# NUSTM/FacialMMT

Hardware: AMD Instinct MI355X
Metric: utterances/sec T+A+V forward+bwd, 160-frame face seq, 1/2/4/8 GPU (higher is better)
Workload: dtype bf16; 1 GPU; configs[1]: T+A+V, RoBERTa-large (random init), 160-frame face seq (uint8 112x112 crops, fused pil-bicubic x2 + normalise), batch 4 utterances/GPU, bf16, fwd+bwd+clip+AdamW every step; global_batch=4, parallelism=dp1, hip_graphs=whole step: 2 graphs (fwd+bwd | clip+optimizer), text_encoder_concurrent_with_swin=True, swin_forward_pipelined_across_steps=False, text_encoder_parameters=bf16 with fp32 master weights in the optimizer

## Files before the change

### facialmmt_amd/_lib.py

```python
from __future__ import annotations

import ctypes as C
import os

_HERE = os.path.dirname(os.path.abspath(__file__))
LIB_PATH = os.path.join(_HERE, "libfmmt_hip.so")

F32, BF16 = 0, 1
GENERIC = 0x100
EPI_NONE, EPI_GELU, EPI_GELU_BWD, EPI_GELU_DG, EPI_MUL_AUX = 0, 1, 2, 3, 4
SAVE_DG = 0x200
BATCH_MAJOR = 0x400
RESIZE_PIL, RESIZE_CV2 = 0, 1

_p, _i, _f, _sz, _u64 = C.c_void_p, C.c_int, C.c_float, C.c_size_t, C.c_uint64

SIGNATURES = {
    "fmmt_version": (_i, []),
    "fmmt_linear_fwd": (_i, [_i, _i, _i, _i, _p, _i, _p, _i, _p, _p, _i, _p, _i, _p, _i, _p, _i, _p, _i, _p]),
    "fmmt_linear_splitk_workspace": (_sz, [_i, _i, _i]),
    "fmmt_linear_fwd_splitk": (_i, [_i, _i, _i, _i, _p, _i, _p, _i, _p, _p, _i, _p, _sz, _p]),
    "fmmt_linear_wgrad_workspace": (_sz, [_i, _i, _i, _i]),
    "fmmt_linear_wgrad": (_i, [_i, _i, _i, _i, _p, _i, _p, _i, _p, _p, _p, _i, _i, _p, _sz, _p]),
    "fmmt_linear_wgrad_partials": (_i, [_i, _i, _i, _i, _p, _i, _p, _i, _i, _p, _i, _i, _p, _sz, _p]),
# ... 108 lines not shown

GROUPS_SIGNATURES = {
    "fmmt_adamw_groups": (_i, [_i, _i, _p, _i, _p, _p, _p, _p, _f, _i, _p]),
    "fmmt_adamw_groups_guarded": (_i, [_i, _i, _p, _i, _p, _p, _p, _p, _f, _i, _p]),
}
ADAMW_GROUP_BYTES = 32
ADAMW_GROUP_FIELDS = [("lr", "<u8"), ("beta1", "<f4"), ("beta2", "<f4"), ("eps", "<f4"), ("weight_decay", "<f4"), ("pad", "<u4", (2,))]

STATS_SIGNATURES = {
    "fmmt_table_stats": (_i, [_i, _i, _i, _p, _p, _p, _p, _p, _p, _p]),
}
STATS_G, STATS_P, STATS_M, STATS_V = 0, 1, 2, 3
STATS_BYTES, STATS_BAD_WORDS = 16, 2
STATS_FIELDS = [("sumsq", "<f4"), ("max_abs", "<f4"), ("nonfinite", "<i4"), ("reserved", "<i4")]

TOKENS_SIGNATURES = {
    "fmmt_token_layout": (_i, [_i, _i, _i, _p, _p, _p, _p, _p, _p, _p]),
    "fmmt_unpack_rows": (_i, [_i, _i, _i, _sz, _p, _p, _p, _p]),
    "fmmt_mha_fwd_ragged": (_i, [_i, _i, _i, _i, _i, _i, _p, _p, _p, _i, _p, _p, _i, _f, _f, _u64, _p, _p, _i, _p, _p]),
    "fmmt_mha_bwd_ragged": (_i, [_i, _i, _i, _i, _i, _i, _p, _p, _p, _i, _p, _p, _i, _f, _f, _u64, _p, _p, _p, _i, _p, _p, _i, _p, _p, _i, _p]),
    "fmmt_dropadd_ln_fwd_map": (_i, [_i, _i, _i, _f, _p, _p, _p, _p, _f, _u64, _p, _u64, _p, _p, _p, _p]),
    "fmmt_dropadd_ln_bwd_map": (_i, [_i, _i, _i, _f, _p, _p, _p, _f, _u64, _p, _u64, _p, _p, _p, _p, _p, _p, _sz, _p, _p]),
}
LOSS_SIGNATURES = {
    "fmmt_ce_fwd": (_i, [_i, _i, _i, _p, _i, _p, _p, _f, _p, _p, _p]),
    "fmmt_ce_bwd": (_i, [_i, _i, _i, _p, _i, _p, _p, _f, _p, _p, _p, _i, _p]),
    "fmmt_pool_head_fwd_crit": (_i, [_i, _i, _i, _i, _i, _p, _p, _p, _p, _p, _p, _p, _p, _p, _f, _u64, _p, _p, _p, _p, _p, _p, _p, _f, _p, _p, _sz, _p]),
    "fmmt_pool_head_bwd_crit": (_i, [_i, _i, _i, _i, _i, _p, _p, _p, _p, _p, _p, _p, _p, _p, _p, _p, _p, _f, _p, _p, _p, _p, _p, _p, _p, _p, _p, _sz, _p]),
}
ROUTE_SIGNATURES = {
    "fmmt_linear_fwd_route": (_i, [_i] * 17),
    "fmmt_linear_wgrad_route": (_i, [_i] * 10),
}
ROUTE_MODE_FWD, ROUTE_MODE_SEG3_N, ROUTE_MODE_SEG3_K, ROUTE_MODE_SPLITK = 0, 1, 2, 3
CE_MAXNL, CE_MAXB = 8, 65536
RAGGED = 0x800

FMMT_EINVAL, FMMT_EALIGN, FMMT_EWORKSPACE = -1, -2, -3
_ERR = {-1: "FMMT_EINVAL (bad shape / unsupported size)", -2: "FMMT_EALIGN (pointer or leading dimension not 16-byte aligned)",
        -3: "FMMT_EWORKSPACE (workspace too small)"}

_lib = None


class FmmtError(RuntimeError):
    pass


def load():
    global _lib
    if _lib is not None:
        return _lib
    if not os.path.exists(LIB_PATH):
        raise FmmtError(f"{LIB_PATH} is missing: build it with `python -m facialmmt_amd.build` "
                        f"(or __graft_entry__.build()); there is no CPU / PyTorch fallback for the hot path")
    lib = C.CDLL(LIB_PATH)
    for name, (res, args) in list(SIGNATURES.items()) + list(POOL_HEAD_SIGNATURES.items()) + list(RAGGED_SIGNATURES.items()) + list(EVAL_COLLECT_SIGNATURES.items()) + list(POOL_HEAD_ROWS_SIGNATURES.items()) + list(GUARD_SIGNATURES.items()) + list(DIGEST_SIGNATURES.items()) + list(EVAL_SHARD_SIGNATURES.items()) + list(JITTER_SIGNATURES.items()) + list(AUG_SIGNATURES.items()) + list(GROUPS_SIGNATURES.items()) + list(STATS_SIGNATURES.items()) + list(TOKENS_SIGNATURES.items()) + list(LOSS_SIGNATURES.items()) + list(ROUTE_SIGNATURES.items()):
        fn = getattr(lib, name)
        fn.restype = res
        fn.argtypes = args
    _lib = lib
    return lib


def check(rc: int, what: str):
    if rc != 0:
        msg = _ERR.get(rc, f"hipError_t {rc}")
        raise FmmtError(f"{what} failed: {msg}")


def dtype_code(t) -> int:
    import torch
    if t == torch.float32:
        return F32
    if t == torch.bfloat16:
        return BF16
    raise FmmtError(f"unsupported activation dtype {t}: the HIP path computes in float32 (parity) or bfloat16 (throughput)")
```

### facialmmt_amd/build.py

```python
from __future__ import annotations

import glob
import os
import subprocess
import sys
from concurrent.futures import ThreadPoolExecutor

HERE = os.path.dirname(os.path.abspath(__file__))
CSRC = os.path.join(HERE, "csrc")
OUT = os.path.join(HERE, "libfmmt_hip.so")
SOURCES = ["gemm.hip", "layernorm.hip", "attn.hip", "wattn_mfma.hip", "wattn_bwd_ref.hip", "wblock.hip", "wblock_ref.hip", "mha_mfma.hip", "misc.hip", "preproc.hip", "mlp_fused.hip", "mlp_ref.hip", "patch_ln.hip", "lin_lnbwd.hip", "plm_fused.hip", "frame_filter.hip", "eval.hip", "pool_head.hip", "ragged.hip", "guard.hip", "digest.hip", "eval_shard.hip", "color_jitter.hip", "aff_augment.hip", "adamw_groups.hip", "table_stats.hip", "ce_loss.hip"]
FLAGS = ["--offload-arch=gfx950", "-O3", "-std=c++17", "-fPIC", "-ffp-contract=fast"]


def _stale(target, deps):
    if not os.path.exists(target):
        return True
    t = os.path.getmtime(target)
    return any(os.path.getmtime(d) > t for d in deps)


def build(force: bool = False, verbose: bool = True, tag: str = "") -> str:
    hipcc = os.environ.get("HIPCC", "/opt/rocm/bin/hipcc")
    tag = tag or os.environ.get("FMMT_BUILD_TAG", "")
    csrc = os.environ.get("FMMT_CSRC_DIR", CSRC) if tag else CSRC
    headers = sorted(glob.glob(os.path.join(csrc, "*.h"))) + [os.path.join(csrc, "..", "..", "include", h) for h in ("fmmt.h", "fmmt_pool_head.h", "fmmt_ragged.h", "fmmt_eval_collect.h", "fmmt_pool_head_rows.h", "fmmt_guard.h", "fmmt_digest.h", "fmmt_eval_shard.h", "fmmt_jitter.h", "fmmt_aug.h", "fmmt_groups.h", "fmmt_stats.h", "fmmt_tokens.h", "fmmt_loss.h", "fmmt_route.h")]
    objdir = os.path.join(HERE, "build_" + tag if tag else "build")
    out = os.path.join(HERE, f"libfmmt_hip_{tag}.so") if tag else OUT
    os.makedirs(objdir, exist_ok=True)
    jobs = []
    for s in SOURCES:
        src = os.path.join(csrc, s)
        obj = os.path.join(objdir, s.replace(".hip", ".o"))
        if force or _stale(obj, [src] + headers):
            jobs.append((src, obj))

    def cc(job):
        src, obj = job
        cmd = [hipcc] + FLAGS + os.environ.get("FMMT_CFLAGS", "").split() + ["-c", src, "-o", obj]
        if verbose:
            print(" ".join(cmd), flush=True)
        subprocess.run(cmd, check=True)

    with ThreadPoolExecutor(max_workers=4) as ex:
        list(ex.map(cc, jobs))
    objs = [os.path.join(objdir, s.replace(".hip", ".o")) for s in SOURCES]
    if force or jobs or _stale(out, objs):
        cmd = [hipcc, "--offload-arch=gfx950", "-shared", "-fPIC", "-o", out] + objs
        if verbose:
            print(" ".join(cmd), flush=True)
        subprocess.run(cmd, check=True)
    return out


if __name__ == "__main__":
    print(build(force="--force" in sys.argv))
```

### facialmmt_amd/csrc/misc.hip

```cpp
#include "fmmt_common.h"
#include "bn1d_core.h"
#include "adamw_core.h"
#include "../../include/fmmt.h"

namespace {

constexpr int IMG = 224, PS = 4, GRID = 56, KPATCH = 48;

template <typename T, bool TO_COLS>
__global__ void patch_cols_kernel(const T* __restrict__ src, T* __restrict__ dst, size_t total) {
    const size_t t = (size_t)blockIdx.x * blockDim.x + threadIdx.x;
    if (t >= total) return;
    const int px = (int)(t % GRID);
    size_t r = t / GRID;
    const int y = (int)(r % IMG);
    r /= IMG;
    const int c = (int)(r % 3);
    const size_t n = r / 3;
    const size_t img_off = ((n * 3 + c) * IMG + y) * IMG + (size_t)px * PS;
    const size_t col_off = ((n * GRID + (y >> 2)) * GRID + px) * KPATCH + c * 16 + (y & 3) * PS;
    const T* s = TO_COLS ? src + img_off : src + col_off;
    T* d = TO_COLS ? dst + col_off : dst + img_off;
    if constexpr (sizeof(T) == 2) *reinterpret_cast<uint2*>(d) = *reinterpret_cast<const uint2*>(s);
    else *reinterpret_cast<uint4*>(d) = *reinterpret_cast<const uint4*>(s);
// ... 147 lines not shown
    }
#pragma unroll
    for (int i = 0; i < 4; ++i) {
        const int r = tr * 64 + ty + 16 * i;
#pragma unroll
        for (int j = 0; j < 4; ++j) {
            const int c = tc * 64 + tx + 16 * j;
            if (r < d.rows && c < d.cols) {
                const size_t o = (size_t)r * d.src_ld + c;
                const bf16 v = f32 ? (bf16)sf[o] : sb[o];
                if (tp) tile[ty + 16 * i][tx + 16 * j] = v;
                else dst[(size_t)r * d.cols + c] = v;
            }
        }
    }
    if (!tp) return;
    __syncthreads();
#pragma unroll
    for (int i = 0; i < 4; ++i) {
        const int c = tc * 64 + ty + 16 * i;
#pragma unroll
        for (int j = 0; j < 4; ++j) {
            const int r = tr * 64 + tx + 16 * j;
            if (r < d.rows && c < d.cols) dst[(size_t)c * d.rows + r] = tile[tx + 16 * j][ty + 16 * i];
        }
    }
}

struct HoDesc {
    const void* src; float* dst;
    long long n;
    int blk_begin, flags;
};
__global__ __launch_bounds__(256) void grad_handover_kernel(const HoDesc* __restrict__ desc, int n_desc, float* __restrict__ partial) {
    __shared__ float red[4];
    int lo = 0, hi = n_desc - 1;
    while (lo < hi) {
        const int mid = (lo + hi + 1) >> 1;
        if (desc[mid].blk_begin <= (int)blockIdx.x) lo = mid;
        else hi = mid - 1;
    }
    const HoDesc d = desc[lo];
    const long long base = (long long)((int)blockIdx.x - d.blk_begin) * 4096;
    const bool bf = d.flags & 1, acc = d.flags & 2;
    const float* sf = reinterpret_cast<const float*>(d.src);
    const bf16* sb = reinterpret_cast<const bf16*>(d.src);
    float ss = 0.f;
    const bool vec = base + 4096 <= d.n && ((reinterpret_cast<uintptr_t>(d.src) | reinterpret_cast<uintptr_t>(d.dst)) & 15) == 0;
    if (vec) {
#pragma unroll
        for (int i = 0; i < 4; ++i) {
            const long long o = base + (long long)(i * 256 + threadIdx.x) * 4;
            f32x4 v;
            if (bf) {
                const bf16x4 t = *reinterpret_cast<const bf16x4*>(sb + o);
#pragma unroll
                for (int e = 0; e < 4; ++e) v[e] = (float)t[e];
            } else {
                v = *reinterpret_cast<const f32x4*>(sf + o);
            }
            if (acc) v += *reinterpret_cast<const f32x4*>(d.dst + o);
            *reinterpret_cast<f32x4*>(d.dst + o) = v;
#pragma unroll
            for (int e = 0; e < 4; ++e) ss += v[e] * v[e];
        }
    } else {
        for (long long o = base + threadIdx.x; o < base + 4096 && o < d.n; o += 256) {
            float v = bf ? (float)sb[o] : sf[o];
            if (acc) v += d.dst[o];
            d.dst[o] = v;
            ss += v * v;
        }
    }
    ss = wave_sum(ss);
    if ((threadIdx.x & 63) == 0) red[threadIdx.x >> 6] = ss;
    __syncthreads();
    if (threadIdx.x == 0) partial[blockIdx.x] = (red[0] + red[1]) + (red[2] + red[3]);
}
__global__ __launch_bounds__(1024) void sumsq_finish_kernel(const float* __restrict__ partial, int n, float* __restrict__ out) {
    __shared__ float red[1024];
    float a = 0.f;
    int i = threadIdx.x;
    for (; i + 7 * 1024 < n; i += 8 * 1024) {
        float v[8];
#pragma unroll
        for (int u = 0; u < 8; ++u) v[u] = partial[i + u * 1024];
#pragma unroll
        for (int u = 0; u < 8; ++u) a += v[u];
    }
    for (; i < n; i += 1024) a += partial[i];
    red[threadIdx.x] = a;
    __syncthreads();
    for (int s = 512; s > 0; s >>= 1) {
        if ((int)threadIdx.x < s) red[threadIdx.x] += red[threadIdx.x + s];
        __syncthreads();
    }
    if (threadIdx.x == 0) out[0] = sqrtf(red[0]);
}

__global__ __launch_bounds__(256) void adamw_batch_kernel(const AdamDesc* __restrict__ desc, int n_desc, const float* __restrict__ lr_p,
                                                          const float* __restrict__ step_p, const float* __restrict__ norm_p,
                                                          float beta1, float beta2, float eps, float wd, float max_norm, int hf) {
    const int r = adamw_find_record(desc, n_desc);
    adamw_batch_body<false>(desc[r], AdamHyper{*lr_p, beta1, beta2, eps, wd}, step_p, norm_p, max_norm, hf);
}

__global__ __launch_bounds__(256) void lnp_bwd_kernel(int M, int C, float eps, const bf16* __restrict__ dy, const bf16* __restrict__ x,
                                                      const bf16* __restrict__ gamma, bf16* __restrict__ dx, float* __restrict__ part) {
    constexpr int MAXV = 4;
    __shared__ float red[4][2][64 * 8];
// ... 188 lines not shown
    const int vec = dtype == FMMT_BF16 ? 8 : 4;
    if (N % vec || ldx % vec) return FMMT_EINVAL;
    if ((reinterpret_cast<uintptr_t>(x) & 15) != 0) return FMMT_EALIGN;
    hipStream_t st = reinterpret_cast<hipStream_t>(stream);
    const dim3 grid((unsigned)((N + 4 * vec - 1) / (4 * vec)));
    if (dtype == FMMT_BF16) {
        if (out_dtype == FMMT_BF16) hipLaunchKernelGGL((colsum_kernel<bf16, bf16>), grid, dim3(256), 0, st, M, N, (const bf16*)x, ldx, (bf16*)out);
        else hipLaunchKernelGGL((colsum_kernel<bf16, float>), grid, dim3(256), 0, st, M, N, (const bf16*)x, ldx, (float*)out);
    } else {
        hipLaunchKernelGGL((colsum_kernel<float, float>), grid, dim3(256), 0, st, M, N, (const float*)x, ldx, (float*)out);
    }
    FMMT_CHECK_LAUNCH();
    return 0;
}

extern "C" int fmmt_cast_batch(int n_desc, int n_tiles, const void* desc, void* stream) {
    if (n_desc <= 0 || n_tiles <= 0 || !desc) return FMMT_EINVAL;
    hipLaunchKernelGGL(cast_batch_kernel, dim3((unsigned)n_tiles), dim3(256), 0, reinterpret_cast<hipStream_t>(stream),
                       reinterpret_cast<const CastDesc*>(desc), n_desc);
    FMMT_CHECK_LAUNCH();
    return 0;
}

extern "C" int fmmt_grad_handover(int n_desc, int n_blocks, const void* desc, float* partial, float* norm_out, void* stream) {
    if (n_desc <= 0 || n_blocks <= 0 || !desc || !partial || !norm_out) return FMMT_EINVAL;
    hipStream_t st = reinterpret_cast<hipStream_t>(stream);
    hipLaunchKernelGGL(grad_handover_kernel, dim3((unsigned)n_blocks), dim3(256), 0, st, reinterpret_cast<const HoDesc*>(desc), n_desc, partial);
    FMMT_CHECK_LAUNCH();
    hipLaunchKernelGGL(sumsq_finish_kernel, dim3(1), dim3(1024), 0, st, (const float*)partial, n_blocks, norm_out);
    FMMT_CHECK_LAUNCH();
    return 0;
}

extern "C" int fmmt_adamw_batch(int n_desc, int n_blocks, const void* desc, const float* lr, const float* step, const float* total_norm,
                                float beta1, float beta2, float eps, float weight_decay, float max_norm, int hf_semantics, void* stream) {
    if (n_desc <= 0 || n_blocks <= 0 || !desc || !lr || !step) return FMMT_EINVAL;
    hipLaunchKernelGGL(adamw_batch_kernel, dim3((unsigned)n_blocks), dim3(256), 0, reinterpret_cast<hipStream_t>(stream),
                       reinterpret_cast<const AdamDesc*>(desc), n_desc, lr, step, total_norm, beta1, beta2, eps, weight_decay, max_norm, hf_semantics);
    FMMT_CHECK_LAUNCH();
    return 0;
}

extern "C" size_t fmmt_layernorm_bwd_bf16_workspace(int M, int C) {
    if (M <= 0 || C <= 0) return 0;
    const int blocks = M / 4 < 1 ? 1 : (M / 4 > 256 ? 256 : M / 4);
    return (size_t)blocks * 2 * (size_t)C * sizeof(float);
}

extern "C" int fmmt_layernorm_bwd_bf16(int M, int C, float eps, const void* dy, const void* x, const void* gamma, void* dx,
                                       void* dgamma, void* dbeta, void* workspace, size_t workspace_bytes, void* stream) {
    if (M <= 0 || C <= 0 || C % 8 || C > 2048) return FMMT_EINVAL;
    if (!dy || !x || !gamma || !dx || !dgamma || !dbeta || !workspace) return FMMT_EINVAL;
    if (workspace_bytes < fmmt_layernorm_bwd_bf16_workspace(M, C)) return FMMT_EWORKSPACE;
    if (((reinterpret_cast<uintptr_t>(dy) | reinterpret_cast<uintptr_t>(x) | reinterpret_cast<uintptr_t>(gamma) | reinterpret_cast<uintptr_t>(dx)) & 15) != 0)
        return FMMT_EALIGN;
    hipStream_t st = reinterpret_cast<hipStream_t>(stream);
    const int blocks = M / 4 < 1 ? 1 : (M / 4 > 256 ? 256 : M / 4);
    hipLaunchKernelGGL(lnp_bwd_kernel, dim3(blocks), dim3(256), 0, st, M, C, eps, (const bf16*)dy, (const bf16*)x, (const bf16*)gamma, (bf16*)dx,
                       reinterpret_cast<float*>(workspace));
    FMMT_CHECK_LAUNCH();
    hipLaunchKernelGGL(lnp_reduce_kernel, dim3((2 * C + 31) / 32), dim3(1024), 0, st, reinterpret_cast<const float*>(workspace), blocks, C,
                       (bf16*)dgamma, (bf16*)dbeta);
    FMMT_CHECK_LAUNCH();
    return 0;
}
```

### facialmmt_amd/ops.py

```python
from __future__ import annotations

import math
import weakref

import torch
from torch.autograd import Function

from . import _lib
from ._lib import EPI_GELU, EPI_GELU_BWD, EPI_GELU_DG, EPI_MUL_AUX, EPI_NONE, SAVE_DG, check, dtype_code


def _st():
    return torch.cuda.current_stream().cuda_stream


def _p(t):
    return None if t is None else t.data_ptr()


def _c16(t: torch.Tensor) -> torch.Tensor:
    t = t.contiguous()
    return t.clone() if t.data_ptr() % 16 else t


# ... 275 lines not shown

def adamw_batch_guarded(n, blocks, desc, lr, step, total_norm, beta1, beta2, eps, weight_decay, max_norm, hf=False):
    if total_norm is None:
        raise ValueError("adamw_batch_guarded: total_norm is what the guard decides on; it cannot be None")
    check(_lib.load().fmmt_adamw_batch_guarded(n, blocks, _p(desc), _p(lr), _p(step), _p(total_norm), float(beta1), float(beta2), float(eps),
                                               float(weight_decay), float(max_norm), 1 if hf else 0, _st()), "fmmt_adamw_batch_guarded")


def _group_tables(n, n_groups, group_of, groups, what):
    if group_of.dtype != torch.int32 or not group_of.is_contiguous() or group_of.numel() != n:
        raise ValueError(f"{what}: group_of is a contiguous int32 tensor with one entry per descriptor record ({n})")
    if groups.dtype != torch.uint8 or not groups.is_contiguous() or groups.numel() != n_groups * _lib.ADAMW_GROUP_BYTES or n_groups < 1:
        raise ValueError(f"{what}: groups is a contiguous uint8 tensor of n_groups >= 1 records of {_lib.ADAMW_GROUP_BYTES} bytes (include/fmmt_groups.h)")
    return _p(group_of), _p(groups)


def adamw_groups(n, blocks, desc, n_groups, group_of, groups, step, total_norm, max_norm, hf=False):
    go, gr = _group_tables(n, n_groups, group_of, groups, "adamw_groups")
    check(_lib.load().fmmt_adamw_groups(n, blocks, _p(desc), n_groups, go, gr, _p(step), _p(total_norm), float(max_norm), 1 if hf else 0, _st()),
          "fmmt_adamw_groups")


def adamw_groups_guarded(n, blocks, desc, n_groups, group_of, groups, step, total_norm, max_norm, hf=False):
    if total_norm is None:
        raise ValueError("adamw_groups_guarded: total_norm is what the guard decides on; it cannot be None")
    go, gr = _group_tables(n, n_groups, group_of, groups, "adamw_groups_guarded")
    check(_lib.load().fmmt_adamw_groups_guarded(n, blocks, _p(desc), n_groups, go, gr, _p(step), _p(total_norm), float(max_norm), 1 if hf else 0,
                                                _st()), "fmmt_adamw_groups_guarded")


def grad_handover_raw(n, blocks, table, partial, norm_out):
    check(_lib.load().fmmt_grad_handover(n, blocks, _p(table), _p(partial), _p(norm_out), torch.cuda.current_stream(table.device).cuda_stream),
          f"fmmt_grad_handover(n={n},blocks={blocks})")


def _guard_words(words):
    if words.dtype != torch.int64 or not words.is_contiguous() or words.numel() != _lib.GUARD_WORDS:
        raise ValueError(f"words: a contiguous int64 tensor of {_lib.GUARD_WORDS} entries (include/fmmt_guard.h)")
    return _p(words)


def guard_commit(total_norm, step, words):
    check(_lib.load().fmmt_guard_commit(_p(total_norm), _p(step), _guard_words(words), _st()), "fmmt_guard_commit")


def monitor_loss(loss, scale, words):
    if loss.dtype != torch.float32 or loss.numel() != 1:
        raise ValueError("monitor_loss: one float32 value on the device")
    check(_lib.load().fmmt_monitor_loss(_p(loss), float(scale), _guard_words(words), _st()), "fmmt_monitor_loss")


def param_digest(n, blocks, desc, out=None, partial=None):
    if out is None:
        out = torch.empty(6, dtype=torch.int64, device=desc.device)
    elif out.dtype != torch.int64 or not out.is_contiguous() or out.numel() != 6:
        raise ValueError("param_digest: out is a contiguous int64 tensor of six entries")
    if partial is None:
        partial = torch.empty(6 * max(int(blocks), 1), dtype=torch.int64, device=desc.device)
    elif partial.dtype != torch.int64 or not partial.is_contiguous() or partial.numel() < 6 * blocks:
        raise ValueError("param_digest: partial is a contiguous int64 tensor of at least 6 * blocks entries")
    check(_lib.load().fmmt_param_digest(n, blocks, _p(desc), _p(partial), _p(out), _st()), "fmmt_param_digest")
    return out


def _stats_rows(t, rows, what):
    if t.dtype != torch.int32 or not t.is_contiguous() or t.dim() != 2 or t.shape[1] != 4 or t.shape[0] < rows:
# ... 1730 lines not shown
```

### facialmmt_amd/train_step.py

```python
from __future__ import annotations

import types

import torch
import torch.nn.functional as F

from .graph_capture import (_KEEP_GRAPHS, _bump_versions, _reset_optimizer_state, capture_window, copy_into_static,
                            distinct_stream, pick_concurrent_stream, replay_update, require_packet_capture_off, warmup_undone)
from . import step_state
from .step_state import StepState


SELECT_FRAMES_KERNEL = True


def select_frames(preds, vision_inputs, vision_mask, num_imgs, threshold, n_valid=None):
    B, Lv, D = vision_inputs.shape
    dev = preds.device
    nF = preds.shape[0]
    if SELECT_FRAMES_KERNEL and torch.is_tensor(num_imgs):
        from . import ops
        if ops.select_frames_fusable(preds, vision_inputs, vision_mask):
            return ops.select_frames(preds, vision_inputs, vision_mask, num_imgs, threshold, n_valid)
    n = torch.as_tensor(num_imgs).to(dev).long()
# ... 464 lines not shown
            self.opt.step()
            if self.sched is not None:
                self.sched.step()
            if averager is not None:
                averager.zero_grad()
            else:
                self.opt.zero_grad(set_to_none=True)
            mark("optimizer")
        self.swin.zero_grad(set_to_none=True)
        return loss.detach(), new_mask


class VendorLinear(torch.nn.Linear):

    def forward(self, x):
        if self.bias is None or not x.is_cuda or x.dtype != self.weight.dtype or x.dtype not in (torch.bfloat16, torch.float32) \
                or self.weight.shape[0] % 8 or not torch.is_grad_enabled():
            return super().forward(x)
        from . import ops
        return ops.VendorLinearFn.apply(x, self.weight, self.bias)


class VendorLayerNorm(torch.nn.LayerNorm):

    def forward(self, x):
        if (self.weight is None or self.bias is None or not x.is_cuda or x.dtype != torch.bfloat16 or self.weight.dtype != torch.bfloat16
                or len(self.normalized_shape) != 1 or x.shape[-1] % 8 or x.shape[-1] > 2048 or not torch.is_grad_enabled()):
            return super().forward(x)
        from . import ops
        return ops.PlmLayerNormFn.apply(x, self.weight, self.bias, self.eps)


PLM_COLSUM, PLM_LN, FUSED_ADAMW, PIN_SHADOWS, FUSED_HANDOVER = True, True, True, True, True
PLM_FUSE_EMBED = True
PLM_FUSE_FFN = True
PLM_FUSE_ATTN = True
PLM_FUSE_TAILS, PLM_FUSE_QKV = True, True


class fused_inference:
    depth = 0

    def __enter__(self):
        fused_inference.depth += 1
        return self

    def __exit__(self, *exc):
        fused_inference.depth -= 1
        return False


def _fusable_now():
    return torch.is_grad_enabled() or fused_inference.depth > 0


def use_colsum_bias_gradients(module):
    if not PLM_COLSUM:
        return 0
    n = 0
    ln = PLM_LN
    for m in module.modules():
        if type(m) is torch.nn.Linear and m.bias is not None:
            m.__class__ = VendorLinear
            n += 1
        elif ln and type(m) is torch.nn.LayerNorm and m.elementwise_affine and m.bias is not None:
            m.__class__ = VendorLayerNorm
# ... 434 lines not shown
                g["lr"] = old["lr"]
                with torch.no_grad():
                    g["lr"].fill_(float(saved))
            for k, v in old.items():
                if k not in g:
                    g[k] = v
            if n is not None:
                if torch.is_tensor(old.get("step")):
                    g["step"] = old["step"]
                    with torch.no_grad():
                        g["step"].fill_(float(n))
                else:
                    g["step"] = torch.full((), float(n), dtype=torch.float32, device=g["params"][0].device)

    def hf_state_dict(self):
        sd = self.state_dict()
        for g in sd["param_groups"]:
            t = g.pop("step", None)
            n = int(t.item()) if torch.is_tensor(t) else int(t or 0)
            for i in g["params"]:
                if i in sd["state"]:
                    sd["state"][i] = dict(sd["state"][i], step=n)
        return sd


class FusedHandOver:

    def __init__(self, n_records: int, captures: int = 4):
        self.hosts = [torch.empty(32 * max(1, n_records), dtype=torch.uint8).pin_memory() for _ in range(2)]
        self.capture_hosts = [torch.empty(32 * max(1, n_records), dtype=torch.uint8).pin_memory() for _ in range(max(1, int(captures)))]
        self.captures = 0
        self.calls = 0
        self.keep = []

    @torch.no_grad()
    def __call__(self, pairs, flat_view_of, accumulate: bool, norm_out) -> bool:
        import numpy as np
        from . import ops
        grads = []
        for p, master in pairs:
            g = p.grad
            if g is None or not g.is_cuda or not g.is_contiguous() or g.dtype not in (torch.float32, torch.bfloat16) or g.numel() != flat_view_of[master].numel():
                return False
            grads.append(g)
        if not grads:
            return False
        dev = grads[0].device
        arr = np.zeros(len(grads), dtype=np.dtype([("src", "<u8"), ("dst", "<u8"), ("n", "<i8"), ("bb", "<i4"), ("flags", "<i4")]))
        blocks = 0
        for i, (g, (p, master)) in enumerate(zip(grads, pairs)):
            arr[i] = (g.data_ptr(), flat_view_of[master].data_ptr(), g.numel(), blocks, (1 if g.dtype == torch.bfloat16 else 0) | (2 if accumulate else 0))
            blocks += (g.numel() + 4095) // 4096
        raw = torch.from_numpy(arr.view(np.uint8))
        if raw.numel() > self.hosts[0].numel():
            return False
        if torch.cuda.is_current_stream_capturing():
            if self.captures >= len(self.capture_hosts):
                raise RuntimeError("FusedHandOver: more captures than pinned capture tables")
            host = self.capture_hosts[self.captures][:raw.numel()]
            self.captures += 1
        else:
            torch.cuda.current_stream(dev).synchronize()
            host = self.hosts[self.calls % 2][:raw.numel()]
            self.calls += 1
        host.copy_(raw)
        table = torch.empty(raw.numel(), dtype=torch.uint8, device=dev)
        table.copy_(host, non_blocking=True)
        partial = torch.empty(blocks, dtype=torch.float32, device=dev)
        ops.grad_handover_raw(len(grads), blocks, table, partial, norm_out)
        self.keep = self.keep[-3:] + [(table, partial)]
        for p, _ in pairs:
            p.grad = None
        return True


class TrainMonitor:

    def __init__(self, device="cuda"):
        from . import _lib
        self.words = torch.zeros(_lib.GUARD_WORDS, dtype=torch.int64, device=device)

    def reset(self):
        self.words.zero_()

    @staticmethod
    def summarise(host_words):
        import numpy as np
        from . import _lib
        host = np.ascontiguousarray(host_words, dtype=np.int64)
        if host.shape != (_lib.GUARD_WORDS,):
            raise ValueError(f"TrainMonitor.summarise: {_lib.GUARD_WORDS} int64 words")
        loss_sum = float(host[_lib.GUARD_LOSS_SUM:_lib.GUARD_LOSS_SUM + 1].view(np.float64)[0])
        micro = int(host[_lib.GUARD_MICRO_STEPS])
        last_norm = float(host[_lib.GUARD_LAST_NORM:_lib.GUARD_LAST_NORM + 1].astype(np.uint32).view(np.float32)[0])
        return types.SimpleNamespace(avg_loss=loss_sum / micro if micro else float("nan"), loss_sum=loss_sum, micro_steps=micro,
                                     nonfinite_losses=int(host[_lib.GUARD_NONFINITE_LOSSES]), applied=int(host[_lib.GUARD_APPLIED]),
                                     skipped=int(host[_lib.GUARD_SKIPPED]), last_norm=last_norm)

    def read(self):
        return self.summarise(self.words.cpu().numpy())

    def loss(self, loss, scale):
# ... 120 lines not shown
            g = opt.param_groups[0]
            self.lr, (self.b1, self.b2), self.eps, self.wd = g["lr"], g["betas"], g["eps"], g["weight_decay"]
        else:
            self.plan = group_plan(opt, params)
        self.hf = isinstance(opt, HFAdamW)
        self.max_norm = float(max_norm)
        dev = params[0].device
        self.step = torch.zeros((), dtype=torch.float32, device=dev)
        self.grads = [grad_of[p] for p in params]
        self.m = [torch.zeros_like(p) for p in params]
        self.v = [torch.zeros_like(p) for p in params]
        self.norm = torch.zeros((), dtype=torch.float32, device=dev)
        self.norm_ready = False
        self.norm_table = self.norm_partial = None
        if FUSED_HANDOVER:
            tb = np.zeros(len(params), dtype=np.dtype([("src", "<u8"), ("dst", "<u8"), ("n", "<i8"), ("bb", "<i4"), ("flags", "<i4")]))
            nb = 0
            for i, g in enumerate(self.grads):
                tb[i] = (g.data_ptr(), g.data_ptr(), g.numel(), nb, 0)
                nb += (g.numel() + 4095) // 4096
            self.norm_table = torch.from_numpy(tb.view(np.uint8).copy()).to(dev)
            self.norm_partial = torch.empty(nb, dtype=torch.float32, device=dev)
            self.norm_blocks = nb
        recs, blocks = [], 0
        self.keep = (params, [low_of.get(id(p)) for p in params])
        for p, gr, m, v, low in zip(params, self.grads, self.m, self.v, self.keep[1]):
            assert gr.dtype == torch.float32 and gr.is_contiguous() and p.is_contiguous() and (low is None or (low.dtype == torch.bfloat16 and low.is_contiguous()))
            recs.append((p.data_ptr(), gr.data_ptr(), m.data_ptr(), v.data_ptr(), low.data_ptr() if low is not None else 0, p.numel(), blocks, 0))
            blocks += (p.numel() + 4095) // 4096
        arr = np.zeros(len(recs), dtype=np.dtype([("p", "<u8"), ("g", "<u8"), ("m", "<u8"), ("v", "<u8"), ("low", "<u8"), ("n", "<i8"), ("bb", "<i4"), ("pad", "<i4")]))
        for i, r in enumerate(recs):
            arr[i] = r
        self.desc = torch.from_numpy(arr.view(np.uint8).copy()).to(dev)
        self.n, self.blocks = len(recs), blocks
        self._digest_partial = None
        if report is not None:
            report.bind(self.desc, self.n, self.blocks, params)
        if self.plan is not None:
            self.group_of, self.group_table = group_tables(self.plan, dev)

    def digest(self, out=None):
        from . import ops
        if self._digest_partial is None:
            self._digest_partial = torch.empty(6 * self.blocks, dtype=torch.int64, device=self.desc.device)
        return ops.param_digest(self.n, self.blocks, self.desc, out=out, partial=self._digest_partial)

    def reset(self):
        self.step.zero_()
        torch._foreach_zero_(self.m)
        torch._foreach_zero_(self.v)

    @torch.no_grad()
    def load_from(self, opt):
        params = self.keep[0]
        plan = self.plan
        hyper = plan.groups if plan is not None else [{"betas": (self.b1, self.b2), "eps": self.eps, "weight_decay": self.wd}]
        group_of = plan.group_of if plan is not None else [0] * len(params)
        if len(opt.param_groups) != len(hyper):
            raise ValueError(f"FusedClipAdamW.load_from: {len(opt.param_groups)} parameter groups loaded, the update was built over {len(hyper)}")
        for j, (g, h) in enumerate(zip(opt.param_groups, hyper)):
            who = "FusedClipAdamW.load_from" if plan is None else f"FusedClipAdamW.load_from, group {j}"
            step_state.check_hyper(g, {k: h[k] for k in ("betas", "eps", "weight_decay")}, who)
        counts = {}
        for j in sorted(set(group_of)):
            t = opt.param_groups[j].get("step")
            ts = {float(t)} if t is not None else {float(opt.state[p]["step"]) for p, k in zip(params, group_of)
                                                   if k == j and p in opt.state and "step" in opt.state[p]}
            if len(ts) > 1:
                raise ValueError(f"per-parameter step counters disagree: {sorted(ts)}")
            counts[j] = ts.pop() if ts else None
        seen = {t for t in counts.values() if t is not None}
        if len(seen) > 1:
            raise ValueError(f"FusedClipAdamW.load_from: the groups' step counters disagree ({counts}); the fused update keeps one counter for all groups")
        for p, m, v in zip(params, self.m, self.v):
            st = opt.state.get(p, {})
            if "exp_avg" in st:
                m.copy_(st["exp_avg"])
                v.copy_(st["exp_avg_sq"])
            else:
                m.zero_()
                v.zero_()
        self.step.fill_(seen.pop() if seen else 0.0)

    @torch.no_grad()
    def export(self, params=None):
        at = {id(p): i for i, p in enumerate(self.keep[0])}
        order = [at[id(p)] for p in (self.keep[0] if params is None else params)]
        return [step_state.to_host(self.m[i]) for i in order], [step_state.to_host(self.v[i]) for i in order], int(self.step.item())

    @torch.no_grad()
    def update(self):
        from . import ops
        if self.monitor is None:
            self.step.add_(1.0)
        if not self.norm_ready:
            if self.norm_table is not None:
                ops.grad_handover_raw(len(self.grads), self.norm_blocks, self.norm_table, self.norm_partial, self.norm)
            else:
                self.norm.copy_(torch.nn.utils.get_total_norm(self.grads, 2.0, foreach=True))
        self.norm_ready = False
        if self.report is not None:
            self.report.record(self.norm)
        if self.group_table is not None:
            n_groups = len(self.plan.groups)
            if self.monitor is not None:
                ops.adamw_groups_guarded(self.n, self.blocks, self.desc, n_groups, self.group_of, self.group_table, self.step, self.norm, self.max_norm, self.hf)
                ops.guard_commit(self.norm, self.step, self.monitor.words)
                return
            ops.adamw_groups(self.n, self.blocks, self.desc, n_groups, self.group_of, self.group_table, self.step, self.norm, self.max_norm, self.hf)
            return
        if self.monitor is not None:
            ops.adamw_batch_guarded(self.n, self.blocks, self.desc, self.lr, self.step, self.norm, self.b1, self.b2, self.eps, self.wd, self.max_norm, self.hf)
            ops.guard_commit(self.norm, self.step, self.monitor.words)
            return
        ops.adamw_batch(self.n, self.blocks, self.desc, self.lr, self.step, self.norm, self.b1, self.b2, self.eps, self.wd, self.max_norm, self.hf)


def _pin_shadows(modules):
    if not PIN_SHADOWS:
        return None
    from . import ops
    seen, params = set(), []
    for m in modules:
        for p in m.parameters():
            if id(p) not in seen:
                seen.add(id(p))
                params.append(p)
    return ops.PinnedShadows(params)


class FlatGradientTail:

    def __init__(self, flat, opt, clip, accumulate, masters=None, exchanging=False, capture_tables=4, monitor=None, report=None):
        from .parallel import GradientAverager
        if not isinstance(flat, GradientAverager):
            flat = list(flat)
        if report is not None and not FusedClipAdamW.eligible(opt, flat.params if isinstance(flat, GradientAverager) else flat):
            raise ValueError("grad_report needs the fused update (FusedClipAdamW.eligible: torch.optim.AdamW / HFAdamW whose parameter groups all hold a "
                             "device learning rate, over fp32 device parameters): the report runs over its descriptor table")
        self.report = report
        if monitor is not None and not FusedClipAdamW.eligible(opt, flat.params if isinstance(flat, GradientAverager) else flat):
            raise ValueError("skip_nonfinite needs the fused update (FusedClipAdamW.eligible: torch.optim.AdamW / HFAdamW whose parameter groups all hold a "
                             "device learning rate, over fp32 device parameters): the stock optimizer path cannot skip an update without a host synchronisation")
        self.monitor = monitor
        self.opt, self.clip, self.accumulate, self.masters, self.exchanging = opt, clip, bool(accumulate), masters, bool(exchanging)
        self.flat = flat if isinstance(flat, GradientAverager) else GradientAverager(flat, hooks=False)
        self.flat_view_of = {p: p.grad for p in self.flat.params}
        low_of = {id(m): l for l, m in (masters.pairs() if masters is not None else [])}
        self.pairs = [(low_of.get(id(p), p), p) for p in self.flat.params]
        for l, m in self.pairs:
            l.grad = None
        self.fused = None
        if FusedClipAdamW.eligible(opt, self.flat.params):
            self.fused = FusedClipAdamW(opt, self.flat.params, self.flat_view_of, low_of, clip, monitor=monitor, report=report)
        self.handover = FusedHandOver(len(self.pairs), captures=capture_tables) if (self.fused is not None and FUSED_HANDOVER) else None

    def hand_over(self):
        ran = self.handover is not None and self.handover(self.pairs, self.flat_view_of, self.accumulate, self.fused.norm)
        if not ran:
            _hand_over_gradients(self.pairs, self.flat_view_of, self.accumulate)
        if self.fused is not None:
            self.fused.norm_ready = ran and not self.exchanging

    def update(self):
        if self.fused is not None:
            self.fused.update()
        else:
            for p in self.flat.params:
                p.grad = self.flat_view_of[p]
            torch.nn.utils.clip_grad_norm_(self.flat.params, self.clip)
            self.opt.step()
            if self.masters is not None:
                self.masters.sync_low()
        if self.accumulate:
            self.flat.zero_grad()
        for l, _ in self.pairs:
            l.grad = None

    def replica_digest(self):
        if self.fused is None:
            raise ValueError("replica_digest needs the fused update (FusedClipAdamW.eligible: torch.optim.AdamW / HFAdamW whose parameter groups all hold a "
                             "device learning rate, over fp32 device parameters): the digest runs over its descriptor table")
        return self.fused.digest()

    def undo_warmup(self):
        _reset_optimizer_state(self.opt)
        if self.fused is not None:
            self.fused.reset()
        self.flat.zero_grad()
        if self.monitor is not None:
            self.monitor.reset()
        if self.report is not None:
            self.report.reset()

    def require_single_rank(self, what):
        if self.flat.active:
            raise NotImplementedError(f"{what}: one rank only (not with an active gradient exchange: per-rank generator state is not saved)")

    def optimizer_state(self):
        if self.fused is None:
            return step_state.stock_optimizer_state(self.opt)
        return step_state.optimizer_state(self.opt, *self.fused.export(step_state.optimizer_params(self.opt)))

    def window(self):
        return [step_state.to_host(self.flat_view_of[p]) for p in step_state.optimizer_params(self.opt)]

    def check_window(self, who):
        if any(p not in self.flat_view_of for p in step_state.optimizer_params(self.opt)):
            raise RuntimeError(f"{who}: the optimizer steps a parameter the flat gradient buffers do not hold")

    @torch.no_grad()
    def load(self, optimizer, window):
        step_state.load_optimizer_state(optimizer, self.opt, self.fused)
        if window is None:
            self.flat.zero_grad()
        else:
            for p, src in zip(step_state.optimizer_params(self.opt), window):
                self.flat_view_of[p].copy_(src)
        for l, _ in self.pairs:
            l.grad = None


class GraphedTargetStep(StepState):

    STATE_KIND, STATE_MODELS, STATE_WINDOW = TargetStep.STATE_KIND, TargetStep.STATE_MODELS, TargetStep.STATE_WINDOW

    TEXT_FORK_AT = "start"

    def __init__(self, swin_model, multimodal_model, optimizer, scheduler, args, batch, autocast_dtype=None,
                 overlap_text=True, parallel_fusion=False, averager=None, warmup_iters=2, masters=None, discarded_swin_gradients="compute",
                 swin_cut: int = 0, pipeline_swin: bool = False, branch_graphs: bool = False, fork_streams: bool = False, frame_capacity=None,
                 pad_rows: bool = False, skip_nonfinite: bool = False, color_jitter=None, grad_report: bool = False, token_capacity=None,
                 criterion=None):
        from . import ops
        from .parallel import GradientAverager
        if discarded_swin_gradients not in ("compute", "skip"):
            raise ValueError("discarded_swin_gradients: 'compute' or 'skip'")
        other_mode = bool(pipeline_swin or branch_graphs or fork_streams)
        box = token_box(multimodal_model)
        if token_capacity is None:
            token_capacity = 0 if (other_mode or box is None) else default_token_capacity(batch[1])
        self.token_capacity = int(token_capacity)
        if self.token_capacity and box is None:
            raise ValueError("token_capacity: the text encoder is not the fused bf16 encoder (MasterWeights / fuse_text_encoder) that can run on packed rows")
        if self.token_capacity < 0:
            raise ValueError("token_capacity: a number of rows, 0 (padded layout) or None (from the sample batch)")
# ... 865 lines not shown
```

### include/fmmt.h

```cpp
#ifndef FMMT_H
#define FMMT_H
#include <stddef.h>
#include <stdint.h>

#ifdef __cplusplus
extern "C" {
#endif

#define FMMT_F32 0
#define FMMT_BF16 1
#define FMMT_GENERIC 0x100
#define FMMT_SAVE_DG 0x200
#define FMMT_BATCH_MAJOR 0x400

#define FMMT_EINVAL (-1)
#define FMMT_EALIGN (-2)
#define FMMT_EWORKSPACE (-3)

#define FMMT_EPI_GELU 1
#define FMMT_EPI_GELU_BWD 2
#define FMMT_EPI_GELU_DG 3
#define FMMT_EPI_MUL_AUX 4

int fmmt_version(void);
// ... 157 lines not shown
#define FMMT_RESIZE_PIL 0
#define FMMT_RESIZE_CV2 1
int fmmt_resize_table(int mode, int in_size, int out_size, int32_t* table, float* lut);
int fmmt_resize_band_rows(const int32_t* table, int out_size);
int fmmt_patch_embed_u8(int dtype, int mode, int n_img, int in_size, const void* img_u8, const int32_t* table_dev,
                        const float* lut_dev, void* cols, void* stream);

int fmmt_patch_embed_ln_fwd(int dtype, int M, int C, int K, const void* cols, const void* w, const float* bias, const float* ln_gamma,
                            const float* ln_beta, float eps, void* x_pre, void* y, float* mean, float* rstd, void* stream);

int fmmt_patch_embed_u8_ln_fwd(int dtype, int mode, int n_img, int in_size, const void* img_u8, const int32_t* table_dev, const float* lut_dev,
                               const void* w, const float* bias, const float* ln_gamma, const float* ln_beta, float eps,
                               void* cols, void* x_pre, void* y, float* mean, float* rstd, void* stream);

int fmmt_emotion_head_fwd(int dtype, int N, int K, int H, int NL, const void* feats, int ld, const float* w1, const float* b1, const float* w2,
                          const float* b2, const float* gumbel, float tau, float* preds, float* importance, void* stream);
int fmmt_eval_accumulate(int dtype, int B, int NL, const void* logits, int ld, const int64_t* labels, double* loss_sum, int64_t* count,
                         int64_t* confusion, int32_t* pred, float* logits_out, int64_t out_offset, int64_t out_capacity, void* stream);

#include "fmmt_pool_head.h"
#include "fmmt_ragged.h"
#include "fmmt_eval_collect.h"
#include "fmmt_pool_head_rows.h"
#include "fmmt_guard.h"
#include "fmmt_digest.h"
#include "fmmt_eval_shard.h"
#include "fmmt_jitter.h"
#include "fmmt_aug.h"
#include "fmmt_groups.h"
#include "fmmt_stats.h"
#include "fmmt_tokens.h"
#include "fmmt_loss.h"
#include "fmmt_route.h"

#ifdef __cplusplus
}
#endif
#endif
```

Before: 75.85 utterances/s.

## Let AdamW read per-parameter gradients directly instead of copying into flat buffers

Adds a grad-norm-publish kernel that computes the gradient sum of squares without writing to the flat fp32 gradient buffers, and patches the AdamW descriptor table so each record points at the original gradient tensor (bf16 or fp32). With no accumulation and no gradient exchange, the hand-over now takes this direct path, removing a full write and re-read of every gradient. In exchange it adds state tracking (eager versus captured publishing, restoring the flat descriptor table on reset or load) and keeps the gradient tensors alive, which makes the graph-captured path more fragile.

```diff
diff --git a/facialmmt_amd/_lib.py b/facialmmt_amd/_lib.py
--- a/facialmmt_amd/_lib.py
+++ b/facialmmt_amd/_lib.py
@@ -164,6 +164,9 @@
     "fmmt_linear_fwd_route": (_i, [_i] * 17),
     "fmmt_linear_wgrad_route": (_i, [_i] * 10),
 }
+DIRECT_SIGNATURES = {
+    "fmmt_grad_norm_publish": (_i, [_i, _i, _p, _p, _p, _p, _p]),
+}
 ROUTE_MODE_FWD, ROUTE_MODE_SEG3_N, ROUTE_MODE_SEG3_K, ROUTE_MODE_SPLITK = 0, 1, 2, 3
 CE_MAXNL, CE_MAXB = 8, 65536
 RAGGED = 0x800
@@ -187,7 +190,7 @@
         raise FmmtError(f"{LIB_PATH} is missing: build it with `python -m facialmmt_amd.build` "
                         f"(or __graft_entry__.build()); there is no CPU / PyTorch fallback for the hot path")
     lib = C.CDLL(LIB_PATH)
-    for name, (res, args) in list(SIGNATURES.items()) + list(POOL_HEAD_SIGNATURES.items()) + list(RAGGED_SIGNATURES.items()) + list(EVAL_COLLECT_SIGNATURES.items()) + list(POOL_HEAD_ROWS_SIGNATURES.items()) + list(GUARD_SIGNATURES.items()) + list(DIGEST_SIGNATURES.items()) + list(EVAL_SHARD_SIGNATURES.items()) + list(JITTER_SIGNATURES.items()) + list(AUG_SIGNATURES.items()) + list(GROUPS_SIGNATURES.items()) + list(STATS_SIGNATURES.items()) + list(TOKENS_SIGNATURES.items()) + list(LOSS_SIGNATURES.items()) + list(ROUTE_SIGNATURES.items()):
+    for name, (res, args) in list(SIGNATURES.items()) + list(POOL_HEAD_SIGNATURES.items()) + list(RAGGED_SIGNATURES.items()) + list(EVAL_COLLECT_SIGNATURES.items()) + list(POOL_HEAD_ROWS_SIGNATURES.items()) + list(GUARD_SIGNATURES.items()) + list(DIGEST_SIGNATURES.items()) + list(EVAL_SHARD_SIGNATURES.items()) + list(JITTER_SIGNATURES.items()) + list(AUG_SIGNATURES.items()) + list(GROUPS_SIGNATURES.items()) + list(STATS_SIGNATURES.items()) + list(TOKENS_SIGNATURES.items()) + list(LOSS_SIGNATURES.items()) + list(ROUTE_SIGNATURES.items()) + list(DIRECT_SIGNATURES.items()):
         fn = getattr(lib, name)
         fn.restype = res
         fn.argtypes = args
diff --git a/facialmmt_amd/build.py b/facialmmt_amd/build.py
--- a/facialmmt_amd/build.py
+++ b/facialmmt_amd/build.py
@@ -24,7 +24,7 @@
     hipcc = os.environ.get("HIPCC", "/opt/rocm/bin/hipcc")
     tag = tag or os.environ.get("FMMT_BUILD_TAG", "")
     csrc = os.environ.get("FMMT_CSRC_DIR", CSRC) if tag else CSRC
-    headers = sorted(glob.glob(os.path.join(csrc, "*.h"))) + [os.path.join(csrc, "..", "..", "include", h) for h in ("fmmt.h", "fmmt_pool_head.h", "fmmt_ragged.h", "fmmt_eval_collect.h", "fmmt_pool_head_rows.h", "fmmt_guard.h", "fmmt_digest.h", "fmmt_eval_shard.h", "fmmt_jitter.h", "fmmt_aug.h", "fmmt_groups.h", "fmmt_stats.h", "fmmt_tokens.h", "fmmt_loss.h", "fmmt_route.h")]
+    headers = sorted(glob.glob(os.path.join(csrc, "*.h"))) + [os.path.join(csrc, "..", "..", "include", h) for h in ("fmmt.h", "fmmt_pool_head.h", "fmmt_ragged.h", "fmmt_eval_collect.h", "fmmt_pool_head_rows.h", "fmmt_guard.h", "fmmt_digest.h", "fmmt_eval_shard.h", "fmmt_jitter.h", "fmmt_aug.h", "fmmt_groups.h", "fmmt_stats.h", "fmmt_tokens.h", "fmmt_loss.h", "fmmt_route.h", "fmmt_direct.h")]
     objdir = os.path.join(HERE, "build_" + tag if tag else "build")
     out = os.path.join(HERE, f"libfmmt_hip_{tag}.so") if tag else OUT
     os.makedirs(objdir, exist_ok=True)
diff --git a/facialmmt_amd/csrc/misc.hip b/facialmmt_amd/csrc/misc.hip
--- a/facialmmt_amd/csrc/misc.hip
+++ b/facialmmt_amd/csrc/misc.hip
@@ -203,7 +203,8 @@
     long long n;
     int blk_begin, flags;
 };
-__global__ __launch_bounds__(256) void grad_handover_kernel(const HoDesc* __restrict__ desc, int n_desc, float* __restrict__ partial) {
+template <bool COPY>
+__device__ __forceinline__ void grad_handover_body(const HoDesc* __restrict__ desc, int n_desc, float* __restrict__ partial, AdamDesc* adam) {
     __shared__ float red[4];
     int lo = 0, hi = n_desc - 1;
     while (lo < hi) {
@@ -213,11 +214,12 @@
     }
     const HoDesc d = desc[lo];
     const long long base = (long long)((int)blockIdx.x - d.blk_begin) * 4096;
-    const bool bf = d.flags & 1, acc = d.flags & 2;
+    const bool bf = d.flags & 1, acc = COPY && (d.flags & 2);
     const float* sf = reinterpret_cast<const float*>(d.src);
     const bf16* sb = reinterpret_cast<const bf16*>(d.src);
     float ss = 0.f;
-    const bool vec = base + 4096 <= d.n && ((reinterpret_cast<uintptr_t>(d.src) | reinterpret_cast<uintptr_t>(d.dst)) & 15) == 0;
+    const uintptr_t where = COPY ? reinterpret_cast<uintptr_t>(d.src) | reinterpret_cast<uintptr_t>(d.dst) : reinterpret_cast<uintptr_t>(d.src);
+    const bool vec = base + 4096 <= d.n && (where & 15) == 0;
     if (vec) {
 #pragma unroll
         for (int i = 0; i < 4; ++i) {
@@ -230,23 +232,39 @@
             } else {
                 v = *reinterpret_cast<const f32x4*>(sf + o);
             }
-            if (acc) v += *reinterpret_cast<const f32x4*>(d.dst + o);
-            *reinterpret_cast<f32x4*>(d.dst + o) = v;
+            if constexpr (COPY) {
+                if (acc) v += *reinterpret_cast<const f32x4*>(d.dst + o);
+                *reinterpret_cast<f32x4*>(d.dst + o) = v;
+            }
 #pragma unroll
             for (int e = 0; e < 4; ++e) ss += v[e] * v[e];
         }
     } else {
         for (long long o = base + threadIdx.x; o < base + 4096 && o < d.n; o += 256) {
             float v = bf ? (float)sb[o] : sf[o];
-            if (acc) v += d.dst[o];
-            d.dst[o] = v;
+            if constexpr (COPY) {
+                if (acc) v += d.dst[o];
+                d.dst[o] = v;
+            }
             ss += v * v;
+        }
+    }
+    if constexpr (!COPY) {
+        if (base == 0 && threadIdx.x == 0) {
+            adam[lo].g = d.src;
+            adam[lo].g_bf16 = bf ? 1 : 0;
         }
     }
     ss = wave_sum(ss);
     if ((threadIdx.x & 63) == 0) red[threadIdx.x >> 6] = ss;
     __syncthreads();
     if (threadIdx.x == 0) partial[blockIdx.x] = (red[0] + red[1]) + (red[2] + red[3]);
+}
+__global__ __launch_bounds__(256) void grad_handover_kernel(const HoDesc* __restrict__ desc, int n_desc, float* __restrict__ partial) {
+    grad_handover_body<true>(desc, n_desc, partial, nullptr);
+}
+__global__ __launch_bounds__(256) void grad_norm_publish_kernel(const HoDesc* __restrict__ desc, int n_desc, float* __restrict__ partial, AdamDesc* adam) {
+    grad_handover_body<false>(desc, n_desc, partial, adam);
 }
 __global__ __launch_bounds__(1024) void sumsq_finish_kernel(const float* __restrict__ partial, int n, float* __restrict__ out) {
     __shared__ float red[1024];
@@ -501,6 +519,19 @@
     return 0;
 }
 
+extern "C" int fmmt_grad_norm_publish(int n_desc, int n_blocks, const void* desc, float* partial, float* norm_out, void* adam_desc, void* stream) {
+    if (n_desc <= 0 || n_blocks <= 0 || !desc || !partial || !norm_out || !adam_desc) return FMMT_EINVAL;
+    if (((reinterpret_cast<uintptr_t>(desc) | reinterpret_cast<uintptr_t>(adam_desc)) & 7) != 0) return FMMT_EALIGN;
+    if (((reinterpret_cast<uintptr_t>(partial) | reinterpret_cast<uintptr_t>(norm_out)) & 3) != 0) return FMMT_EALIGN;
+    hipStream_t st = reinterpret_cast<hipStream_t>(stream);
+    hipLaunchKernelGGL(grad_norm_publish_kernel, dim3((unsigned)n_blocks), dim3(256), 0, st, reinterpret_cast<const HoDesc*>(desc), n_desc, partial,
+                       reinterpret_cast<AdamDesc*>(adam_desc));
+    FMMT_CHECK_LAUNCH();
+    hipLaunchKernelGGL(sumsq_finish_kernel, dim3(1), dim3(1024), 0, st, (const float*)partial, n_blocks, norm_out);
+    FMMT_CHECK_LAUNCH();
+    return 0;
+}
+
 extern "C" int fmmt_adamw_batch(int n_desc, int n_blocks, const void* desc, const float* lr, const float* step, const float* total_norm,
                                 float beta1, float beta2, float eps, float weight_decay, float max_norm, int hf_semantics, void* stream) {
     if (n_desc <= 0 || n_blocks <= 0 || !desc || !lr || !step) return FMMT_EINVAL;
diff --git a/facialmmt_amd/ops.py b/facialmmt_amd/ops.py
--- a/facialmmt_amd/ops.py
+++ b/facialmmt_amd/ops.py
@@ -331,6 +331,15 @@
 def grad_handover_raw(n, blocks, table, partial, norm_out):
     check(_lib.load().fmmt_grad_handover(n, blocks, _p(table), _p(partial), _p(norm_out), torch.cuda.current_stream(table.device).cuda_stream),
           f"fmmt_grad_handover(n={n},blocks={blocks})")
+
+
+def grad_norm_publish_raw(n, blocks, table, partial, norm_out, adam_desc):
+    if adam_desc.dtype != torch.uint8 or not adam_desc.is_contiguous() or adam_desc.numel() != 56 * n or adam_desc.device != table.device:
+        raise ValueError(f"grad_norm_publish_raw: adam_desc is adamw_batch's table of {n} records of 56 bytes, on the table's device")
+    if partial.dtype != torch.float32 or not partial.is_contiguous() or partial.numel() < blocks:
+        raise ValueError(f"grad_norm_publish_raw: partial is a contiguous float32 tensor of at least {blocks} entries")
+    check(_lib.load().fmmt_grad_norm_publish(n, blocks, _p(table), _p(partial), _p(norm_out), _p(adam_desc),
+                                             torch.cuda.current_stream(table.device).cuda_stream), f"fmmt_grad_norm_publish(n={n},blocks={blocks})")
 
 
 def _guard_words(words):
diff --git a/facialmmt_amd/train_step.py b/facialmmt_amd/train_step.py
--- a/facialmmt_amd/train_step.py
+++ b/facialmmt_amd/train_step.py
@@ -520,6 +520,7 @@
 
 
 PLM_COLSUM, PLM_LN, FUSED_ADAMW, PIN_SHADOWS, FUSED_HANDOVER = True, True, True, True, True
+DIRECT_UPDATE = True
 PLM_FUSE_EMBED = True
 PLM_FUSE_FFN = True
 PLM_FUSE_ATTN = True
@@ -1020,9 +1021,11 @@
         self.captures = 0
         self.calls = 0
         self.keep = []
+        self.held = None
+        self.capture_grads = []
 
     @torch.no_grad()
-    def __call__(self, pairs, flat_view_of, accumulate: bool, norm_out) -> bool:
+    def __call__(self, pairs, flat_view_of, accumulate: bool, norm_out, publish_to=None) -> bool:
         import numpy as np
         from . import ops
         grads = []
@@ -1055,7 +1058,16 @@
         table = torch.empty(raw.numel(), dtype=torch.uint8, device=dev)
         table.copy_(host, non_blocking=True)
         partial = torch.empty(blocks, dtype=torch.float32, device=dev)
-        ops.grad_handover_raw(len(grads), blocks, table, partial, norm_out)
+        if publish_to is None:
+            ops.grad_handover_raw(len(grads), blocks, table, partial, norm_out)
+            self.held = None
+        else:
+            if accumulate:
+                raise ValueError("FusedHandOver: publish_to leaves the flat buffers alone; an accumulation window needs them")
+            ops.grad_norm_publish_raw(len(grads), blocks, table, partial, norm_out, publish_to)
+            self.held = grads
+            if torch.cuda.is_current_stream_capturing():
+                self.capture_grads.append(grads)
         self.keep = self.keep[-3:] + [(table, partial)]
         for p, _ in pairs:
             p.grad = None
@@ -1242,6 +1254,9 @@
         for i, r in enumerate(recs):
             arr[i] = r
         self.desc = torch.from_numpy(arr.view(np.uint8).copy()).to(dev)
+        self.desc_flat = self.desc.clone()
+        self.published = None
+        self.ever_published = False
         self.n, self.blocks = len(recs), blocks
         self._digest_partial = None
         if report is not None:
@@ -1299,8 +1314,23 @@
         return [step_state.to_host(self.m[i]) for i in order], [step_state.to_host(self.v[i]) for i in order], int(self.step.item())
 
     @torch.no_grad()
+    def use_flat_gradients(self):
+        if self.published is not None:
+            self.norm_ready = False
+        self.published = None
+        if self.ever_published:
+            self.desc.copy_(self.desc_flat)
+
+    @torch.no_grad()
     def update(self):
         from . import ops
+        capturing = self.desc.is_cuda and torch.cuda.is_current_stream_capturing()
+        if capturing and self.published == "eager":
+            raise RuntimeError("FusedClipAdamW.update under capture behind an eager publishing hand-over: capture the hand-over as well")
+        if self.published != ("capture" if capturing else "eager"):
+            self.use_flat_gradients()
+        if not capturing:
+            self.published = None
         if self.monitor is None:
             self.step.add_(1.0)
         if not self.norm_ready:
@@ -1364,13 +1394,21 @@
         if FusedClipAdamW.eligible(opt, self.flat.params):
             self.fused = FusedClipAdamW(opt, self.flat.params, self.flat_view_of, low_of, clip, monitor=monitor, report=report)
         self.handover = FusedHandOver(len(self.pairs), captures=capture_tables) if (self.fused is not None and FUSED_HANDOVER) else None
+        self.direct = bool(DIRECT_UPDATE and self.handover is not None and not self.accumulate and not self.exchanging)
+        self.paths = {"direct": 0, "flat": 0}
 
     def hand_over(self):
-        ran = self.handover is not None and self.handover(self.pairs, self.flat_view_of, self.accumulate, self.fused.norm)
+        ran = self.handover is not None and self.handover(self.pairs, self.flat_view_of, self.accumulate, self.fused.norm,
+                                                          publish_to=self.fused.desc if self.direct else None)
         if not ran:
             _hand_over_gradients(self.pairs, self.flat_view_of, self.accumulate)
         if self.fused is not None:
             self.fused.norm_ready = ran and not self.exchanging
+            self.fused.published = None
+            if ran and self.direct:
+                self.fused.published = "capture" if torch.cuda.is_current_stream_capturing() else "eager"
+                self.fused.ever_published = True
+        self.paths["direct" if ran and self.direct else "flat"] += 1
 
     def update(self):
         if self.fused is not None:
@@ -1397,6 +1435,7 @@
         _reset_optimizer_state(self.opt)
         if self.fused is not None:
             self.fused.reset()
+            self.fused.use_flat_gradients()
         self.flat.zero_grad()
         if self.monitor is not None:
             self.monitor.reset()
@@ -1422,6 +1461,8 @@
     @torch.no_grad()
     def load(self, optimizer, window):
         step_state.load_optimizer_state(optimizer, self.opt, self.fused)
+        if self.fused is not None:
+            self.fused.use_flat_gradients()
         if window is None:
             self.flat.zero_grad()
         else:
diff --git a/include/fmmt.h b/include/fmmt.h
--- a/include/fmmt.h
+++ b/include/fmmt.h
@@ -213,6 +213,7 @@
 #include "fmmt_tokens.h"
 #include "fmmt_loss.h"
 #include "fmmt_route.h"
+#include "fmmt_direct.h"
 
 #ifdef __cplusplus
 }
diff --git a/include/fmmt_direct.h b/include/fmmt_direct.h
--- /dev/null
+++ b/include/fmmt_direct.h
@@ -0,0 +1,15 @@
+#ifndef FMMT_DIRECT_H
+#define FMMT_DIRECT_H
+#include <stddef.h>
+#include <stdint.h>
+
+#ifdef __cplusplus
+extern "C" {
+#endif
+
+int fmmt_grad_norm_publish(int n_desc, int n_blocks, const void* desc, float* partial, float* norm_out, void* adam_desc, void* stream);
+
+#ifdef __cplusplus
+}
+#endif
+#endif
```

Measured after the change: 76.44 utterances/s, median of 6. Within noise of the previous version (+0.8%).
